# AbrahamSanders/realtime-codec-agent

Hardware: AMD Instinct MI355X
Metric: batch-encode audio-hours/hour (+ xRT and p50 frame-step latency of 1 duplex stream in `duplex`) (higher is better)
Workload: dtype f32; 1 GPU; batch MagiCodec-style encode, 16 kHz stereo, 0.1 s chunks / 2.0 s context, 256 windows per step (BASELINE configs[1]); codebook=131072x16

## Files before the change

realtime_codec_agent_amd/csrc/rca_codec.hip:

```cpp
#include <stdarg.h>

#include <algorithm>
#include <array>
#include <cmath>
#include <map>
#include <type_traits>

#include "rca_common.h"
#include "rca_conv_balance.h"

namespace rca {
thread_local char g_err[512] = {0};
}
using namespace rca;

typedef float f32x16 __attribute__((ext_vector_type(16)));

#define RCA_LAT_MAX_FRAMES 64
#define RCA_LDS_BUDGET (152 * 1024)

typedef float f32x4 __attribute__((ext_vector_type(4)));

struct RowSrc {
    const float* base;
    int C;
    long chan_stride;
    long win_stride;
    int T;
    const long* row_off = nullptr;
    long span = 0;
    __device__ __forceinline__ long off(long b) const {
        return row_off ? row_off[b] : (b % C) * chan_stride + (b / C) * win_stride;
    }
};

__device__ __forceinline__ float lrelu(float v, float slope) { return v >= 0.0f ? v : v * slope; }

template <int KS>
__global__ __launch_bounds__(256) void conv_in_kernel(RowSrc src, const float* __restrict__ w,
// ... 136 lines not shown
        const int d = TR ? -kk : kk - padL;
        return (d >= 0) ? d / S : -((-d + S - 1) / S);
    }
    static constexpr int off(int kp, int half, int U) {
        const int kl = 2 * kp + half, ci = kl / KS, kk = kl % KS;
        const int d = TR ? -kk : kk - padL;
        const int q = q_of(kp, half);
        return (ci * S + (d - q * S)) * U + 1 + q;
    }
    static constexpr int delta(int kp, int U) { return off(kp, 1, U) - off(kp, 0, U); }
    static constexpr int distinct(int k, int KPC, int U) {
        int found[4] = {0, 0, 0, 0};
        int n = 0;
        for (int kp = 0; kp < KPC; ++kp) {
            const int d = delta(kp, U);
            bool seen = false;
            for (int i = 0; i < n; ++i) seen = seen || found[i] == d;
            if (!seen && n < 4) found[n++] = d;
        }
        return found[k < n ? k : n - 1];
    }
    static constexpr int count(int KPC, int U) {
        int found[8] = {0, 0, 0, 0, 0, 0, 0, 0};
        int n = 0;
        for (int kp = 0; kp < KPC; ++kp) {
            const int d = delta(kp, U);
            bool seen = false;
            for (int i = 0; i < n; ++i) seen = seen || found[i] == d;
            if (!seen && n < 8) found[n++] = d;
        }
        return n;
    }
};

#ifndef RCA_CONV_WPB
#define RCA_CONV_WPB 1
#endif
#ifndef RCA_CONV_OCC
#define RCA_CONV_OCC 2
#endif
#ifndef RCA_CONV_PIPE
#define RCA_CONV_PIPE 1
#endif
#ifndef RCA_CONV_PRIO
#define RCA_CONV_PRIO 1
#endif
#ifndef RCA_CONV_ABUF
#define RCA_CONV_ABUF 1
#endif
#ifndef RCA_CONV_EPRIO
#define RCA_CONV_EPRIO 1
#endif
#ifdef RCA_ABL_NOBREAD
#define RCA_ABL_BREAD(x) (slope)
#else
#define RCA_ABL_BREAD(x) (x)
#endif
typedef __bf16 conv_bf16x8 __attribute__((ext_vector_type(8)));
typedef __bf16 conv_bf16x2 __attribute__((ext_vector_type(2)));
__device__ __forceinline__ unsigned conv_pack_bf16x2(float a, float b) {
    const conv_bf16x2 v = {(__bf16)a, (__bf16)b};
    return __builtin_bit_cast(unsigned, v);
}
template <int BF>
__device__ __forceinline__ void conv_split8(const float (&w)[8], uint4& hi, uint4& lo) {
    unsigned ph[4], pl[4];
#pragma unroll
    for (int j = 0; j < 4; ++j) {
        ph[j] = conv_pack_bf16x2(w[2 * j], w[2 * j + 1]);
        pl[j] = BF == 3 ? conv_pack_bf16x2(w[2 * j] - __uint_as_float(ph[j] << 16), w[2 * j + 1] - __uint_as_float(ph[j] & 0xffff0000u)) : 0u;
    }
    hi = make_uint4(ph[0], ph[1], ph[2], ph[3]);
    lo = make_uint4(pl[0], pl[1], pl[2], pl[3]);
}
template <int KS, int S, int CIC, int WM, int WN, int FUSE, int TR, int BF, int FULLC>
__device__ __forceinline__ void conv1d_mfma_body(const float* __restrict__ x, const float* __restrict__ wp,
                                                 const float* __restrict__ bias, float* __restrict__ y,
                                                 int Cin, int Lin, int Cout, int Lout, long Ncols, int nchunks,
                                                 int pre, float slope, FuseIn fin, TrInfo tr, const long wg, const long n_off) {
    constexpr int MT = WM * 32;
    constexpr int NW = WN * 32;
    constexpr int U = ConvLds<S>::stride(NW);
    constexpr int KPC = CIC * KS / 2;
    constexpr int QPC = KPC / 4;
    constexpr int E = (NW + 2) * S;
    constexpr int PW = (S % 2 == 0 && !TR) ? 2 : 1;
    constexpr int RE = (E + 64 * PW - 1) / (64 * PW);
    constexpr int padL = (KS - S + 1) / 2;
    constexpr int BUF = CIC * S * U + 4;
    static_assert((CIC * KS) % 8 == 0, "chunk must hold whole weight quads");

    extern __shared__ __attribute__((aligned(16))) float xs_all[];
#ifdef RCA_CONV_TIMELINE
    long* const tl_buf = rca_prof_buf;
#endif
    RCA_TL_STAMP(tl0);

    const int lane = threadIdx.x & 63;
    const int half = lane >> 5;
    const int wave = __builtin_amdgcn_readfirstlane(threadIdx.x >> 6);
    float* xs = xs_all + wave * 2 * BUF;
    const int n_co_real = (Cout + MT - 1) / MT;
    const int n_co = TR ? n_co_real * tr.s : n_co_real;
    const int xcd = (int)(wg & 7);
    const long seq = wg >> 3;
    const int co_tile_x = __builtin_amdgcn_readfirstlane((int)(seq % n_co));
    const int phase = TR ? co_tile_x / n_co_real : 0;
    const int co_tile = TR ? co_tile_x % n_co_real : co_tile_x;
    const long col_tile = (seq / n_co) * 8 + xcd;
    const long n0 = n_off + (col_tile * RCA_CONV_WPB + wave) * NW;
    const int co0 = co_tile * MT;
    if (n0 >= Ncols) return;
    const long n_base = n0 > 0 ? n0 - 1 : 0;
    const int b_base = __builtin_amdgcn_readfirstlane((int)((unsigned)n_base / (unsigned)Lout));
    const int t_base = (int)(n_base - (long)b_base * Lout);
    const int lead = n0 > 0 ? 0 : 1;
    const long left = Ncols - n_base;
    const int ncol_left = left > NW + 2 ? NW + 2 : (int)left;
    auto rel_bt = [&](int dn, int& bb, int& tt) {
        int dt = dn + t_base;
        bb = 0;
        if (Lout >= NW + 3) {
            if (dt >= Lout) { dt -= Lout; bb = 1; }
        } else {
            bb = dt / Lout;
            dt -= bb * Lout;
        }
        tt = dt;
    };

    constexpr unsigned OOB = 0x80000000u;
    const rca_rsrc_t rs_x = rca_make_rsrc(FUSE ? fin.src.base : x + (long)b_base * Cin * Lin, 0x7FFFFFFF);
// ... 99 lines not shown
    float4 a[WM][QPC];
    if (!FUSE) stage_load(0);
#pragma unroll
    for (int wm = 0; wm < WM; ++wm) {
        const float4* p0 = w_ptr(wm, 0);
#pragma unroll
        for (int q = 0; q < QPC; ++q) a[wm][q] = RCA_CONV_ABUF ? w_load(wm, 0, q) : p0[q * 64];
    }
    __builtin_amdgcn_sched_barrier(0);
    typedef ConvBOff<KS, S, TR> BO;
    static_assert(BO::count(KPC, U) <= 3, "B-operand base registers");
    constexpr int BD0 = BO::distinct(0, KPC, U), BD1 = BO::distinct(1, KPC, U), BD2 = BO::distinct(2, KPC, U);
    const int b_base0 = (lane & 31) + half * BD0, b_base1 = (lane & 31) + half * BD1, b_base2 = (lane & 31) + half * BD2;
    auto b_off = [&](int kp) __attribute__((always_inline)) {
        const int dl = BO::delta(kp, U);
        return (dl == BD0 ? b_base0 : dl == BD1 ? b_base1 : b_base2) + BO::off(kp, 0, U);
    };
    unsigned m_first = 0, m_last = 0;
#pragma unroll
    for (int kp = 0; kp < KPC; ++kp) {
        const int q = half ? BO::q_of(kp, 1) : BO::q_of(kp, 0);
        if (q < 0) m_first |= 1u << kp;
        if (q > 0) m_last |= 1u << kp;
    }
    unsigned zmask[WN];
    unsigned zany = 0;
#pragma unroll
    for (int wn = 0; wn < WN; ++wn) {
        int bz, t;
        rel_bt(1 - lead + wn * 32 + (lane & 31), bz, t);
        zmask[wn] = (t == 0 ? m_first : 0u) | (t == Lout - 1 ? m_last : 0u);
        zany |= zmask[wn];
    }
    const bool edges = __builtin_amdgcn_ballot_w64(zany != 0) != 0;

    f32x16 acc[WM][WN];
#pragma unroll
    for (int wm = 0; wm < WM; ++wm) {
#pragma unroll
        for (int q = 0; q < 4; ++q) {
            const f32x4 bq = *reinterpret_cast<const f32x4*>(bias + co0 + wm * 32 + 8 * q + 4 * half);
#pragma unroll
            for (int j = 0; j < 4; ++j)
#pragma unroll
                for (int wn = 0; wn < WN; ++wn) acc[wm][wn][4 * q + j] = bq[j];
        }
    }

    auto stage_write_t = [&](int buf, auto act_tag) __attribute__((always_inline)) {
        constexpr bool ACT = decltype(act_tag)::value;
#ifdef RCA_ABL_NOWRITE
        return;
#endif
        float* dst = xs + buf * BUF;
#pragma unroll
        for (int cl = 0; cl < CIC; ++cl) {
#pragma unroll
            for (int r = 0; r < RE; ++r) {
                float v[PW];
#pragma unroll
                for (int j = 0; j < PW; ++j) {
                    v[j] = sreg[cl][r][j];
                    if (ACT && !FUSE) v[j] = fmaxf(v[j], v[j] * slope);
                }
                if (U > NW + 2 || 64 * PW * (r + 1) <= E || s_loff[r] >= 0) {
#pragma unroll
                    for (int j = 0; j < PW; ++j) dst[cl * S * U + s_loff[r] + j * U] = v[j];
                }
            }
        }
    };
    auto stage_write = [&](int buf) __attribute__((always_inline)) {
        if (pre & 1) stage_write_t(buf, std::true_type{});
        else stage_write_t(buf, std::false_type{});
    };

    auto compute_t = [&](int buf, int cn, auto edge_tag) __attribute__((always_inline)) {
        constexpr bool EDGE = decltype(edge_tag)::value;
        const float* xb = xs + buf * BUF;
        const float4* pn[WM];
#pragma unroll
        for (int wm = 0; wm < WM; ++wm) pn[wm] = w_ptr(wm, cn);
        constexpr int NB = (KPC * WN > 32) ? ((KPC % 4 == 0) ? 4 : 2) : (KPC * WN == 32 && WN == 4) ? 2 : 1;
        constexpr int PB = KPC / NB;
        static_assert(KPC % NB == 0, "batching");
#pragma unroll
        for (int nb = 0; nb < NB; ++nb) {
            float bv[PB][WN];
#pragma unroll
            for (int i = 0; i < PB; ++i)
#pragma unroll
                for (int wn = 0; wn < WN; ++wn) bv[i][wn] = xb[b_off(nb * PB + i) + wn * 32];
#pragma unroll
            for (int i = 0; i < PB; ++i) {
                const int kp = nb * PB + i;
                float bfr[WN];
#pragma unroll
                for (int wn = 0; wn < WN; ++wn) bfr[wn] = (EDGE && ((zmask[wn] >> kp) & 1u)) ? 0.0f : bv[i][wn];
#pragma unroll
                for (int wm = 0; wm < WM; ++wm) {
                    const float4 q4 = a[wm][kp >> 2];
                    const float av = (kp & 3) == 0 ? q4.x : (kp & 3) == 1 ? q4.y : (kp & 3) == 2 ? q4.z : q4.w;
#pragma unroll
                    for (int wn = 0; wn < WN; ++wn)
                        acc[wm][wn] = __builtin_amdgcn_mfma_f32_32x32x2f32(av, bfr[wn], acc[wm][wn], 0, 0, 0);
                }
                if ((kp & 3) == 3) {
#pragma unroll
                    for (int wm = 0; wm < WM; ++wm) a[wm][kp >> 2] = RCA_CONV_ABUF ? w_load(wm, cn, kp >> 2) : pn[wm][(kp >> 2) * 64];
                }
            }
        }
    };

    constexpr bool PIPE = RCA_CONV_PIPE && !TR && KS == 16 && BF == 0;
    constexpr int RD = KPC >= 8 ? 4 : 2;
    float bhead[RD][WN];
    auto read_head = [&](int buf) __attribute__((always_inline)) {
        const float* xb = xs + buf * BUF;
#pragma unroll
        for (int i = 0; i < RD; ++i)
#pragma unroll
            for (int wn = 0; wn < WN; ++wn) bhead[i][wn] = RCA_ABL_BREAD(xb[b_off(i) + wn * 32]);
    };
    auto compute_p = [&](int buf, int cn, auto edge_tag) __attribute__((always_inline)) {
        constexpr bool EDGE = decltype(edge_tag)::value;
        const float* xb = xs + buf * BUF;
        const float4* pn[WM];
#pragma unroll
        for (int wm = 0; wm < WM; ++wm) pn[wm] = w_ptr(wm, cn);
        float ring[KPC][WN];
#pragma unroll
        for (int i = 0; i < RD; ++i)
#pragma unroll
            for (int wn = 0; wn < WN; ++wn) ring[i][wn] = bhead[i][wn];
#pragma unroll
        for (int kp = 0; kp < KPC; ++kp) {
#if RCA_CONV_PRIO
            if (kp == KPC / 4 && !RCA_CONV_EPRIO) __builtin_amdgcn_s_setprio(1);
            if (kp == KPC / 2) __builtin_amdgcn_s_setprio(2);
            if (kp == 3 * KPC / 4) __builtin_amdgcn_s_setprio(3);
#endif
            if (kp + RD < KPC) {
#pragma unroll
                for (int wn = 0; wn < WN; ++wn) ring[kp + RD][wn] = RCA_ABL_BREAD(xb[b_off(kp + RD) + wn * 32]);
            }
            float bfr[WN];
#pragma unroll
// ... 51 lines not shown
                    const conv_bf16x8 bhv = __builtin_bit_cast(conv_bf16x8, bh[wn]);
                    acc[wm][wn] = __builtin_amdgcn_mfma_f32_32x32x16_bf16(ahv, bhv, acc[wm][wn], 0, 0, 0);
                    if (BF == 3) {
                        acc[wm][wn] = __builtin_amdgcn_mfma_f32_32x32x16_bf16(ahv, __builtin_bit_cast(conv_bf16x8, bl[wn]), acc[wm][wn], 0, 0, 0);
                        acc[wm][wn] = __builtin_amdgcn_mfma_f32_32x32x16_bf16(alv, bhv, acc[wm][wn], 0, 0, 0);
                    }
                }
#pragma unroll
                for (int qq = 0; qq < 2; ++qq) {
                    const int q = 2 * g + qq;
                    if (q < QPC) a[wm][q] = w_load(wm, cn, q);
                }
            }
        }
    };

    if (FUSE) stage_load(0);
    stage_write(0);
    __builtin_amdgcn_wave_barrier();
    if constexpr (PIPE) read_head(0);
    RCA_TL_STAMP(tl1);
#ifdef RCA_CONV_TIMELINE
    long tl_load = 1 << 30, tl_mfma = 0, tl_write = 0;
#endif
    const int lastc = nchunks - 1;
    auto chunk_loop = [&](auto edge_tag, auto act_tag) __attribute__((always_inline)) {
    for (int c = 0; c < nchunks; c += 2) {
        const int c1 = min(c + 1, lastc);
        RCA_TL_STAMP(ta);
        stage_load(c1);
        __builtin_amdgcn_sched_barrier(0);
        RCA_TL_STAMP(tb);
        __builtin_amdgcn_s_setprio(RCA_CONV_EPRIO);
        if constexpr (BF != 0) compute_b(0, c1, edge_tag);
        else if constexpr (PIPE) compute_p(0, c1, edge_tag);
        else compute_t(0, c1, edge_tag);
        __builtin_amdgcn_s_setprio(RCA_CONV_PRIO ? 3 : 2);
        __builtin_amdgcn_sched_barrier(0);
        RCA_TL_STAMP(tc);
        stage_write_t(1, act_tag);
        __builtin_amdgcn_wave_barrier();
        if constexpr (PIPE) {
            read_head(1);
            __builtin_amdgcn_sched_barrier(0);
        }
        RCA_TL_STAMP(td);
        RCA_TL_MIN(tl_load, tb, tc); RCA_TL_ADD(tl_mfma, tb, tc); RCA_TL_ADD(tl_write, tc, td);
        if (c + 1 >= nchunks) break;
        const int c2 = min(c + 2, lastc);
        stage_load(c2);
        __builtin_amdgcn_sched_barrier(0);
        __builtin_amdgcn_s_setprio(RCA_CONV_EPRIO);
        if constexpr (BF != 0) compute_b(1, c2, edge_tag);
        else if constexpr (PIPE) compute_p(1, c2, edge_tag);
        else compute_t(1, c2, edge_tag);
        __builtin_amdgcn_s_setprio(RCA_CONV_PRIO ? 3 : 2);
        __builtin_amdgcn_sched_barrier(0);
        stage_write_t(0, act_tag);
        __builtin_amdgcn_wave_barrier();
        if constexpr (PIPE) {
            read_head(0);
            __builtin_amdgcn_sched_barrier(0);
        }
    }
    };
    if (pre & 1) {
        if (edges) chunk_loop(std::true_type{}, std::true_type{});
        else chunk_loop(std::false_type{}, std::true_type{});
    } else {
        if (edges) chunk_loop(std::true_type{}, std::false_type{});
        else chunk_loop(std::false_type{}, std::false_type{});
    }

    if (RCA_CONV_EPRIO) __builtin_amdgcn_s_setprio(0);
    RCA_TL_STAMP(tl2);
    const long orow = TR ? tr.Lout : Lout;
    const bool full_rows = co0 + MT <= Cout;
    float* const yw = y + ((long)b_base * Cout + co0) * orow;
#pragma unroll
    for (int wn = 0; wn < WN; ++wn) {
        const int dn = 1 - lead + wn * 32 + (lane & 31);
        if (dn >= ncol_left) continue;
        int bb, t;
        rel_bt(dn, bb, t);
        int ocol = t;
        if (TR) {
            ocol = tr.s * t - tr.padL + phase;
            if (ocol < 0 || ocol >= (int)orow) continue;
        }
        const unsigned voff = ((unsigned)bb * (unsigned)(Cout * (int)orow) + (unsigned)ocol + (unsigned)(4 * half) * (unsigned)orow) * 4u;
        if (pre & 2) {
#pragma unroll
            for (int wm = 0; wm < WM; ++wm)
#pragma unroll
                for (int r = 0; r < 16; ++r) acc[wm][wn][r] = fmaxf(acc[wm][wn][r], acc[wm][wn][r] * slope);
        }
        if (full_rows) {
#pragma unroll
            for (int wm = 0; wm < WM; ++wm)
#pragma unroll
                for (int r = 0; r < 16; ++r) {
                    const int cu = wm * 32 + (r & 3) + 8 * (r >> 2);
                    char* const yr = reinterpret_cast<char*>(yw + (long)cu * orow);
                    *reinterpret_cast<float*>(yr + voff) = acc[wm][wn][r];
                }
        } else {
#pragma unroll
            for (int wm = 0; wm < WM; ++wm)
#pragma unroll
                for (int r = 0; r < 16; ++r) {
                    const int cu = wm * 32 + (r & 3) + 8 * (r >> 2);
                    char* const yr = reinterpret_cast<char*>(yw + (long)cu * orow);
                    if (co0 + cu + 4 * half < Cout) *reinterpret_cast<float*>(yr + voff) = acc[wm][wn][r];
                }
        }
    }
#ifdef RCA_CONV_TIMELINE
    if (tl_buf && lane == 0) {
        const long tl3 = (long)wall_clock64();
        const unsigned hw = __builtin_amdgcn_s_getreg((31 << 11) | (0 << 6) | 4);
        const unsigned xcc = __builtin_amdgcn_s_getreg((3 << 11) | (0 << 6) | 20);
        constexpr int region = KS == 4 ? 0 : KS == 8 ? 1 : KS == 10 ? 2 : KS == 16 ? 3 : KS == 3 ? 4 : 5;
        long* o = tl_buf + ((long)region * 65536 + ((blockIdx.x * RCA_CONV_WPB + wave) & 0xFFFF)) * 8;
        o[6] = tl_load | (tl_mfma << 32);
        o[7] = tl_write | ((long)nchunks << 32);
        o[0] = tl0; o[1] = tl1; o[2] = tl2; o[3] = tl3;
        o[4] = (long)hw | ((long)xcc << 32);
        o[5] = (long)KS | ((long)S << 8) | ((long)(WM | (WN << 4)) << 16) | ((long)wave << 24) | ((long)blockIdx.x << 32);
    }
#endif
}

template <int KS, int S, int CIC, int WM, int WN, int FUSE, int TR, int BF = 0, int FULLC = 0>
__global__ __launch_bounds__(64 * RCA_CONV_WPB, (((KS == 8 && CIC == 2) || (KS == 16 && CIC == 1)) && WM * WN < 8) ? 3 : RCA_CONV_OCC) void conv1d_mfma_kernel(const float* __restrict__ x, const float* __restrict__ wp,
                                                          const float* __restrict__ bias, float* __restrict__ y,
                                                          int Cin, int Lin, int Cout, int Lout, long Ncols, int nchunks,
                                                          int pre, float slope, FuseIn fin, TrInfo tr) {
    conv1d_mfma_body<KS, S, CIC, WM, WN, FUSE, TR, BF, FULLC>(x, wp, bias, y, Cin, Lin, Cout, Lout, Ncols, nchunks, pre, slope, fin, tr, blockIdx.x, 0);
}

template <int KS, int S, int CIC, int WM, int WN, int WM2, int WN2, int FULLC>
__global__ __launch_bounds__(64 * RCA_CONV_WPB, (((KS == 8 && CIC == 2) || (KS == 16 && CIC == 1)) && WM * WN < 8) ? 3 : RCA_CONV_OCC) void conv1d_mfma_mixed_kernel(const float* __restrict__ x, const float* __restrict__ wp,
                                                          const float* __restrict__ bias, float* __restrict__ y,
                                                          int Cin, int Lin, int Cout, int Lout, long Ncols, int nchunks,
                                                          int pre, float slope, unsigned n_bulk_wg, long fine_col0) {
    const FuseIn fin{};
    const TrInfo tr{};
    if (blockIdx.x < n_bulk_wg) conv1d_mfma_body<KS, S, CIC, WM, WN, 0, 0, 0, FULLC>(x, wp, bias, y, Cin, Lin, Cout, Lout, Ncols, nchunks, pre, slope, fin, tr, blockIdx.x, 0);
    else conv1d_mfma_body<KS, S, CIC, WM2, WN2, 0, 0, 0, FULLC>(x, wp, bias, y, Cin, Lin, Cout, Lout, Ncols, nchunks, pre, slope, fin, tr, blockIdx.x - n_bulk_wg, fine_col0);
}

template <int NWN, bool PRE>
__global__ __launch_bounds__(64, 2) void conv_first_mfma_kernel(const float* __restrict__ wp, const float* __restrict__ bias,
                                                               float* __restrict__ y, int Cout, int Lout, long Ncols, int post, float slope,
                                                               FuseIn fin) {
    constexpr int NW = NWN * 32;
    constexpr int E = (NW + 2) * 2;
    constexpr int NBLK = 2 * NWN + 1;
    constexpr int RS = 136;
    constexpr int ZERO = 128;
    constexpr int CIN = 32, KQ = CIN / 2;
    extern __shared__ __attribute__((aligned(16))) float ring[];
#ifdef RCA_CONV_TIMELINE
    long* const tl_buf = rca_prof_buf;
#endif
    RCA_TL_STAMP(tl0);
    const int lane = threadIdx.x & 63;
    const int half = lane >> 5, jl = lane & 31;
    const int n_co = Cout / 64;
    const long wg = blockIdx.x;
    const int xcd = (int)(wg & 7);
    const long seq = wg >> 3;
    const int co_tile = __builtin_amdgcn_readfirstlane((int)(seq % n_co));
    const long n0 = ((seq / n_co) * 8 + xcd) * NW;
    const int co0 = co_tile * 64;
    if (n0 >= Ncols) return;
    const long n_base = n0 > 0 ? n0 - 1 : 0;
    const int b_base = __builtin_amdgcn_readfirstlane((int)((unsigned)n_base / (unsigned)Lout));
    const int t_base = (int)(n_base - (long)b_base * Lout);
    const int lead = n0 > 0 ? 0 : 1;
    const long left = Ncols - n_base;
    const int ncol_left = left > NW + 2 ? NW + 2 : (int)left;
// ... 878 lines not shown
        out[d.out_off + i] = v;
    }
}

__global__ __launch_bounds__(256) void transpose_fj_kernel(const float* __restrict__ in, float* __restrict__ out, int B,
                                                           int F, int J) {
    const long idx = (long)blockIdx.x * blockDim.x + threadIdx.x;
    if (idx >= (long)B * J * F) return;
    const int f = (int)(idx % F);
    const long r = idx / F;
    const int j = (int)(r % J);
    const int b = (int)(r / J);
    out[idx] = in[((long)b * F + f) * J + j];
}
__global__ __launch_bounds__(256) void transpose_df_kernel(const float* __restrict__ in, float* __restrict__ out, int B,
                                                           int D, int F) {
    const long idx = (long)blockIdx.x * blockDim.x + threadIdx.x;
    if (idx >= (long)B * D * F) return;
    const int d = (int)(idx % D);
    const long r = idx / D;
    const int f = (int)(r % F);
    const int b = (int)(r / F);
    out[idx] = in[((long)b * D + d) * F + f];
}

struct ConvLayer {
    int cin, cout, k, s, pre, tr;
    float* w = nullptr;
    float* b = nullptr;
    float* bp = nullptr;
    float* wp = nullptr;
    int K = 0, Kpad = 0, cout_pad = 0, nchunks = 0;
    float* wp2 = nullptr;
    int nchunks2 = 0;
    float* wp_tr = nullptr;
    float* w_lat = nullptr;
    int nchunks_tr = 0;
};

#ifdef RCA_CONV_SMALLCHUNK
#define RCA_CIC_K8 2
#define RCA_CIC_K16 1
#else
#define RCA_CIC_K8 4
#define RCA_CIC_K16 2
#endif
#ifndef RCA_CIC_K3
#define RCA_CIC_K3 8
#endif
static int conv_cic(int k, int s) {
    if (k == 4 && s == 2) return 4;
    if (k == 8 && s == 4) return RCA_CIC_K8;
    if (k == 10 && s == 5) return 4;
    if (k == 16 && s == 8) return RCA_CIC_K16;
    if (k == 3 && s == 1) return RCA_CIC_K3;
    return 0;
}
static int conv_cic_ws(int k, int s) {
    if (k == 4 && s == 2) return 16;
    if (k == 8 && s == 4) return 8;
    if (k == 10 && s == 5) return 8;
    if (k == 16 && s == 8) return 4;
    if (k == 3 && s == 1) return 16;
    return 0;
}

#ifndef RCA_BLK_ABL
#define RCA_BLK_ABL 0
#endif
typedef unsigned short conv_bf16raw;
typedef __attribute__((ext_vector_type(4))) unsigned conv_u32x4;
// ... 353 lines not shown

static int upload(const rca_tensor_t* ts, int n, const std::string& name, long numel, float** out) {
    const rca_tensor_t* t = find_tensor(ts, n, name);
    if (!t) return fail(RCA_ERR_MISSING, "tensor '%s' missing", name.c_str());
    if (t->numel != numel) return fail(RCA_ERR_ARG, "tensor '%s': numel %ld, expected %ld", name.c_str(), (long)t->numel, numel);
    if (t->dtype != RCA_F32) return fail(RCA_ERR_ARG, "tensor '%s' must be f32", name.c_str());
    RCA_HIP(hipMalloc((void**)out, (size_t)numel * sizeof(float)));
    RCA_HIP(hipMemcpy(*out, t->data, (size_t)numel * sizeof(float), hipMemcpyHostToDevice));
    return RCA_OK;
}

static int pack_weights_cic(const float* w_host, const ConvLayer& L, int cic, float** out, int* nchunks_out) {
    const int K = L.cin * L.k;
    const int nchunks = (L.cin + cic - 1) / cic;
    const int Kpad = nchunks * cic * L.k;
    const int cout_pad = (L.cout + 127) / 128 * 128;
    const long n = (long)(cout_pad / 32) * (Kpad / 8) * 64 * 4;
    std::vector<float> p((size_t)n, 0.0f);
    for (int cot = 0; cot < cout_pad / 32; ++cot)
        for (int q = 0; q < Kpad / 8; ++q)
            for (int lane = 0; lane < 64; ++lane)
                for (int e = 0; e < 4; ++e) {
                    const int co = cot * 32 + (lane & 31);
                    const int k = 2 * (4 * q + e) + (lane >> 5);
                    float v = 0.0f;
                    if (co < L.cout && k < K) v = w_host[(long)co * K + k];
                    p[(((long)cot * (Kpad / 8) + q) * 64 + lane) * 4 + e] = v;
                }
    RCA_HIP(hipMalloc((void**)out, (size_t)n * sizeof(float)));
    RCA_HIP(hipMemcpy(*out, p.data(), (size_t)n * sizeof(float), hipMemcpyHostToDevice));
    *nchunks_out = nchunks;
    return RCA_OK;
}
static int pack_weights(const float* w_host, ConvLayer& L) {
    L.K = L.cin * L.k;
    L.cout_pad = (L.cout + 127) / 128 * 128;
    int rc = pack_weights_cic(w_host, L, conv_cic(L.k, L.s), &L.wp, &L.nchunks);
    if (rc != RCA_OK) return rc;
    L.Kpad = L.nchunks * conv_cic(L.k, L.s) * L.k;
    return pack_weights_cic(w_host, L, conv_cic_ws(L.k, L.s), &L.wp2, &L.nchunks2);
}

static int pack_weights_tr(const float* w_host, ConvLayer& L) {
    const int cic = 16, K = 2 * L.cin;
    const int nchunks = (L.cin + cic - 1) / cic;
    const int Kpad = nchunks * cic * 2;
    L.cout_pad = (L.cout + 127) / 128 * 128;
    const long per_phase = (long)(L.cout_pad / 32) * (Kpad / 8) * 64 * 4;
    std::vector<float> p((size_t)per_phase * L.s, 0.0f);
    for (int r = 0; r < L.s; ++r)
        for (int cot = 0; cot < L.cout_pad / 32; ++cot)
            for (int q = 0; q < Kpad / 8; ++q)
                for (int lane = 0; lane < 64; ++lane)
                    for (int e = 0; e < 4; ++e) {
                        const int co = cot * 32 + (lane & 31);
                        const int k = 2 * (4 * q + e) + (lane >> 5);
                        float v = 0.0f;
                        if (co < L.cout && k < K) {
                            const int ci = k >> 1, j = k & 1;
                            v = w_host[((long)ci * L.cout + co) * L.k + r + j * L.s];
                        }
                        p[r * per_phase + (((long)cot * (Kpad / 8) + q) * 64 + lane) * 4 + e] = v;
                    }
    RCA_HIP(hipMalloc((void**)&L.wp_tr, p.size() * sizeof(float)));
    RCA_HIP(hipMemcpy(L.wp_tr, p.data(), p.size() * sizeof(float), hipMemcpyHostToDevice));
    {
        std::vector<float> t((size_t)L.cin * L.cout * L.k);
        for (int ci = 0; ci < L.cin; ++ci)
            for (int co = 0; co < L.cout; ++co)
                for (int kk = 0; kk < L.k; ++kk) t[((size_t)co * L.k + kk) * L.cin + ci] = w_host[((size_t)ci * L.cout + co) * L.k + kk];
        RCA_HIP(hipMalloc((void**)&L.w_lat, t.size() * sizeof(float)));
        RCA_HIP(hipMemcpy(L.w_lat, t.data(), t.size() * sizeof(float), hipMemcpyHostToDevice));
// ... 19 lines not shown
    RCA_HIP(hipGetDeviceCount(n));
    return RCA_OK;
}

extern "C" int rca_codec_destroy(rca_codec_t* h) {
#ifdef RCA_CONV_TIMELINE
    if (h && getenv("RCA_CONV_TIMELINE_OUT")) {
        long* b = nullptr;
        unsigned n = 6 << 16;
        (void)hipDeviceSynchronize();
        (void)hipMemcpyFromSymbol(&b, HIP_SYMBOL(rca_prof_buf), 8);
        if (b) {
            std::vector<long> host((size_t)(6 << 16) * 8);
            (void)hipMemcpy(host.data(), b, host.size() * 8, hipMemcpyDeviceToHost);
            if (FILE* f = fopen(getenv("RCA_CONV_TIMELINE_OUT"), "wb")) { fwrite(&n, 4, 1, f); fwrite(host.data(), 8, host.size(), f); fclose(f); }
        }
    }
#endif

    if (!h) return RCA_OK;
    (void)hipSetDevice(h->device);
    for (auto& pk : h->bf16_packs) {
        if (pk.hi) (void)hipFree(pk.hi);
        if (pk.lo) (void)hipFree(pk.lo);
        if (pk.w_in8) (void)hipFree(pk.w_in8);
    }
    for (auto* v : {&h->enc, &h->dec})
        for (auto& L : *v) {
            if (L.w) (void)hipFree(L.w);
            if (L.b) (void)hipFree(L.b);
            if (L.bp) (void)hipFree(L.bp);
            if (L.wp) (void)hipFree(L.wp);
            if (L.wp2) (void)hipFree(L.wp2);
            if (L.wp_tr) (void)hipFree(L.wp_tr);
            if (L.w_lat) (void)hipFree(L.w_lat);
        }
    for (float* p : {h->q_in_w, h->q_in_b, h->cb, h->hc, h->cbp})
        if (p) (void)hipFree(p);
    if (h->err_flag) (void)hipFree(h->err_flag);
    for (auto& kv : h->sgraphs)
        if (kv.second.exec) (void)hipGraphExecDestroy(kv.second.exec);
    if (h->pin) (void)hipHostFree(h->pin);
    for (auto& kv : h->ingest_tabs)
        if (kv.second) (void)hipFree(kv.second);
    h->act[0].release(); h->act[1].release(); h->zbuf.release(); h->keys.release(); h->io_a.release(); h->io_b.release(); h->tail.release();
    for (auto* v : {&h->prof, &h->prof_pool})
        for (auto& p : *v) { (void)hipEventDestroy(p.a); (void)hipEventDestroy(p.b); }
    if (h->xev) (void)hipEventDestroy(h->xev);
    if (h->stream) (void)hipStreamDestroy(h->stream);
    delete h;
    return RCA_OK;
}

static void codec_receptive_field(const rca_codec_config_t& c, int hop, int* enc_left, int* dec_left) {
    const int n = c.n_stages;
    long lo = 0;
    lo = lo - (c.k_latent - 1 + 1) / 2;
    for (int i = n - 1; i >= 0; --i) { const int s = c.strides[i], k = 2 * s; lo = lo * s - (k - s + 1) / 2; }
    lo = lo - (c.k_in - 1 + 1) / 2;
    *enc_left = (int)((-lo + hop - 1) / hop);
    auto ceil_div = [](long a, long b) { return a >= 0 ? (a + b - 1) / b : -((-a) / b); };
    long u = 0;
    u = u - (c.k_in - 1 + 1) / 2;
    for (int i = 0; i < n; ++i) { const int s = c.strides[i], k = 2 * s; u = ceil_div(u + (k - s + 1) / 2 - (k - 1), s); }
    u = u - (c.k_latent - 1 + 1) / 2;
    *dec_left = (int)(-u);
// ... 82 lines not shown
    }
#endif
    codebook_proj_kernel<<<cdiv((long)N * J, 256), 256, 0, h->stream>>>(raw, pw, pb, h->cb, N, R, J);
    codebook_norm_pack_kernel<<<cdiv(N, 256), 256, 0, h->stream>>>(h->cb, h->hc, h->cbp, N, J);
    hipError_t e = hipStreamSynchronize(h->stream);
    free3();
    if (e != hipSuccess) return bail(fail(RCA_ERR_HIP, "codebook init: %s", hipGetErrorString(e)));
    *out = h;
    return RCA_OK;
}

extern "C" int rca_codec_hop(const rca_codec_t* h, int32_t* hop) {
    if (!h || !hop) return fail(RCA_ERR_ARG, "null");
    *hop = h->hop;
    return RCA_OK;
}
extern "C" int rca_codec_num_frames(const rca_codec_t* h, int32_t T, int32_t* F) {
    if (!h || !F || T < 0) return fail(RCA_ERR_ARG, "bad argument");
    *F = (T + h->hop - 1) / h->hop;
    return RCA_OK;
}
extern "C" int rca_codec_set_variant(rca_codec_t* h, int32_t v) {
    if (!h || v < 0 || v > 2) return fail(RCA_ERR_ARG, "variant must be 0, 1 or 2");
    h->variant = v;
    return RCA_OK;
}
extern "C" int rca_codec_sync(rca_codec_t* h) {
    if (!h) return fail(RCA_ERR_ARG, "null");
    RCA_HIP(hipSetDevice(h->device));
    RCA_HIP(hipStreamSynchronize(h->stream));
    return RCA_OK;
}

template <int KS, int S, int CIC, int WM, int WN>
static bool launch_conv_balanced(const ConvLayer& L, const float* wp, int nchunks, const float* x, float* y, int Lin, int Lc, long Ncols,
                                 float slope, hipStream_t st, int act, int lds) {
    constexpr int NT = RCA_CONV_WPB * WN * 32, MT = WM * 32;
    const char* on = getenv("RCA_CONV_BALANCE");
    if (on && on[0] == '0') return false;
    const long total = cdiv(Ncols, NT);
    const int n_co = (int)cdiv(L.cout, MT);
    ConvBalancePlan p;
    if (!conv_balance_parse(getenv("RCA_CONV_BALANCE_PLAN"), total, WM, WN, &p)) {
        static int simds_of[64], occ_of[64];
        int dev = 0;
        if (hipGetDevice(&dev) != hipSuccess || dev < 0 || dev >= 64) return false;
        if (!simds_of[dev]) {
            int cus = 0, blocks = 0;
            if (hipDeviceGetAttribute(&cus, hipDeviceAttributeMultiprocessorCount, dev) != hipSuccess || cus <= 0) return false;
            if (hipOccupancyMaxActiveBlocksPerMultiprocessor(&blocks, conv1d_mfma_kernel<KS, S, CIC, WM, WN, 0, 0, 0, 1>, 64 * RCA_CONV_WPB, lds) != hipSuccess || blocks < 4)
                return false;
            occ_of[dev] = blocks * RCA_CONV_WPB / 4;
            simds_of[dev] = 4 * cus;
        }
        p = conv_balance_plan(total, n_co, simds_of[dev], occ_of[dev], WM, WN);
    }
    if (!p.fine_wn) return false;
    const long fine_col0 = p.bulk_col_tiles * NT;
    const long n_bulk_wg = p.bulk_col_tiles * n_co;
    const long fine_tiles = (cdiv(Ncols - fine_col0, RCA_CONV_WPB * p.fine_wn * 32) + 7) / 8 * 8;
    const long n_wg = n_bulk_wg + fine_tiles * cdiv(L.cout, p.fine_wm * 32);
    if (n_wg >= (1L << 31)) return false;
    const dim3 grid((unsigned)n_wg);
    if (WM * WN == 4 && p.fine_wn == 2)
        conv1d_mfma_mixed_kernel<KS, S, CIC, WM, WN, 1, (WM * WN == 4 ? 2 : 1), 1><<<grid, 64 * RCA_CONV_WPB, lds, st>>>(x, wp, L.bp, y, L.cin, Lin, L.cout, Lc, Ncols, nchunks, act, slope, (unsigned)n_bulk_wg, fine_col0);
    else
        conv1d_mfma_mixed_kernel<KS, S, CIC, WM, WN, 1, 1, 1><<<grid, 64 * RCA_CONV_WPB, lds, st>>>(x, wp, L.bp, y, L.cin, Lin, L.cout, Lc, Ncols, nchunks, act, slope, (unsigned)n_bulk_wg, fine_col0);
    return true;
}

template <int KS, int S, int CIC, int WM, int WN, int FUSE, int TR, int BF = 0>
static void launch_conv_cfg(const ConvLayer& L, const float* wp, int nchunks, const float* x, float* y, int Lin, int Lc, long Ncols,
                            float slope, const FuseIn& fin, const TrInfo& tr, hipStream_t st, int act) {
    constexpr int NT = RCA_CONV_WPB * WN * 32, MT = WM * 32;
    constexpr int lds = RCA_CONV_WPB * 2 * (CIC * S * ConvLds<S>::stride(WN * 32) + 4) * 4;
    static_assert(lds <= 65536, "LDS budget");
    const long col_tiles = (cdiv(Ncols, NT) + 7) / 8 * 8;
    dim3 grid((unsigned)(col_tiles * cdiv(L.cout, MT) * (TR ? tr.s : 1)));
    if constexpr (!FUSE && !TR && BF == 0) {
        if (L.cin % CIC == 0 && nchunks * CIC == L.cin) {
            if constexpr (KS >= 8 && WN == 2 && WM <= 2) {
                if (launch_conv_balanced<KS, S, CIC, WM, WN>(L, wp, nchunks, x, y, Lin, Lc, Ncols, slope, st, act, lds)) return;
            }
            conv1d_mfma_kernel<KS, S, CIC, WM, WN, 0, 0, 0, 1><<<grid, 64 * RCA_CONV_WPB, lds, st>>>(x, wp, L.bp, y, L.cin, Lin, L.cout, Lc, Ncols, nchunks, act, slope, fin, tr);
            return;
        }
    }
    conv1d_mfma_kernel<KS, S, CIC, WM, WN, FUSE, TR, BF><<<grid, 64 * RCA_CONV_WPB, lds, st>>>(x, wp, L.bp, y, L.cin, Lin, L.cout, Lc, Ncols, nchunks, act, slope, fin, tr);
}

template <int KS, int S, int CIC>
static int launch_conv_mfma(const ConvLayer& L, const float* x, float* y, int B, int Lin, int Lout, float slope, hipStream_t st,
                            const FuseIn* fuse = nullptr, int act = -1, int bf = 0) {
    if (act < 0) act = L.pre;
    const long Ncols = (long)B * Lout;
    if (bf) {
        const FuseIn none_b{};
        const TrInfo notr_b{};
        const bool big = (long)cdiv(Ncols, 64) * cdiv(L.cout, 64) >= 2048;
#define RCA_BF_LAUNCH(FU, BFM) do { \
            if (big) launch_conv_cfg<KS, S, CIC, 2, 2, FU, 0, BFM>(L, L.wp, L.nchunks, x, y, Lin, Lout, Ncols, slope, FU ? *fuse : none_b, notr_b, st, act); \
            else launch_conv_cfg<KS, S, CIC, 1, 1, FU, 0, BFM>(L, L.wp, L.nchunks, x, y, Lin, Lout, Ncols, slope, FU ? *fuse : none_b, notr_b, st, act); } while (0)
        if constexpr (KS == 4 || KS == 8 || KS == 16) {
            if (fuse) { if (bf == 3) RCA_BF_LAUNCH(1, 3); else RCA_BF_LAUNCH(1, 1); RCA_LAUNCH_CHECK(); return RCA_OK; }
        }
        if (fuse) return fail(RCA_ERR_ARG, "internal: fused first layer of this shape has no bf16 instantiation");
        if (bf == 3) RCA_BF_LAUNCH(0, 3); else RCA_BF_LAUNCH(0, 1);
#undef RCA_BF_LAUNCH
        RCA_LAUNCH_CHECK();
        return RCA_OK;
    }
    const long waves_big = (long)cdiv(Ncols, 64) * cdiv(L.cout, 64);
#ifdef RCA_CONV_FORCE_MID
// ... 1188 lines not shown
```

Before: 3543 audio-hours/hour.

## Add 16x16x4 f32 MFMA path for strided conv layers with repacked weights

Adds an alternative conv1d MFMA body that uses 16x16x4 f32 instructions instead of 32x32x2, with its own B-operand offset classes, edge masks, accumulator layout, epilogue and a separately packed weight buffer. It is selected by default for the k=10, s=5 layers at WM=WN=2 and can be overridden through an env var. The intent is a better fit between the instruction shape and these layers' LDS operand reuse and edge handling. In exchange it costs extra weight memory, more template instantiations, and possibly different register pressure.

Result: no change. 3545 audio-hours/hour, median of 2 (+0.1%).

```diff
diff --git a/realtime_codec_agent_amd/csrc/rca_codec.hip b/realtime_codec_agent_amd/csrc/rca_codec.hip
--- a/realtime_codec_agent_amd/csrc/rca_codec.hip
+++ b/realtime_codec_agent_amd/csrc/rca_codec.hip
@@ -5,6 +5,7 @@
 #include <cmath>
 #include <map>
 #include <type_traits>
+#include <utility>
 
 #include "rca_common.h"
 #include "rca_conv_balance.h"
@@ -207,6 +208,45 @@
         return n;
     }
 };
+
+template <int KS, int S, int KQC, int U>
+struct ConvBOff16 {
+    typedef ConvBOff<KS, S, 0> BO;
+    static constexpr int MAXC = 5;
+    static constexpr int offk(int k) { return BO::off(k >> 1, k & 1, U); }
+    static constexpr int qk(int k) { return BO::q_of(k >> 1, k & 1); }
+    static constexpr int delta(int kq, int g) { return offk(4 * kq + g) - offk(4 * kq); }
+    static constexpr bool same(int a, int b) { return delta(a, 1) == delta(b, 1) && delta(a, 2) == delta(b, 2) && delta(a, 3) == delta(b, 3); }
+    static constexpr int first(int kq) {
+        for (int i = 0; i < kq; ++i) if (same(i, kq)) return i;
+        return kq;
+    }
+    static constexpr int cls(int kq) {
+        int n = 0;
+        const int f = first(kq);
+        for (int i = 0; i < f; ++i) if (first(i) == i) ++n;
+        return n;
+    }
+    static constexpr int count() {
+        int n = 0;
+        for (int i = 0; i < KQC; ++i) if (first(i) == i) ++n;
+        return n;
+    }
+    static constexpr int rep(int c) {
+        int n = 0, last = 0;
+        for (int i = 0; i < KQC; ++i) if (first(i) == i) { if (n == c) return i; ++n; last = i; }
+        return last;
+    }
+    static constexpr unsigned edge_mask(int g, int sign) {
+        unsigned m = 0;
+        for (int kq = 0; kq < KQC; ++kq) if (sign < 0 ? qk(4 * kq + g) < 0 : qk(4 * kq + g) > 0) m |= 1u << kq;
+        return m;
+    }
+};
+template <class F, int... I>
+__device__ __forceinline__ void conv_static_for_impl(F&& f, std::integer_sequence<int, I...>) { (f(std::integral_constant<int, I>{}), ...); }
+template <int N, class F>
+__device__ __forceinline__ void conv_static_for(F&& f) { conv_static_for_impl(f, std::make_integer_sequence<int, N>{}); }
 
 #ifndef RCA_CONV_WPB
 #define RCA_CONV_WPB 1
@@ -248,7 +288,7 @@
     hi = make_uint4(ph[0], ph[1], ph[2], ph[3]);
     lo = make_uint4(pl[0], pl[1], pl[2], pl[3]);
 }
-template <int KS, int S, int CIC, int WM, int WN, int FUSE, int TR, int BF, int FULLC>
+template <int KS, int S, int CIC, int WM, int WN, int FUSE, int TR, int BF, int FULLC, int SH = 32>
 __device__ __forceinline__ void conv1d_mfma_body(const float* __restrict__ x, const float* __restrict__ wp,
                                                  const float* __restrict__ bias, float* __restrict__ y,
                                                  int Cin, int Lin, int Cout, int Lout, long Ncols, int nchunks,
@@ -264,6 +304,9 @@
     constexpr int padL = (KS - S + 1) / 2;
     constexpr int BUF = CIC * S * U + 4;
     static_assert((CIC * KS) % 8 == 0, "chunk must hold whole weight quads");
+    static_assert(SH == 32 || (SH == 16 && !FUSE && !TR && BF == 0 && FULLC == 1), "the 16x16x4 shape covers the plain f32 path only");
+    constexpr int KQC = KPC / 2;
+    constexpr int WM16 = SH == 16 ? 2 * WM : 1, WN16 = SH == 16 ? 2 * WN : 1;
 
     extern __shared__ __attribute__((aligned(16))) float xs_all[];
 #ifdef RCA_CONV_TIMELINE
@@ -273,6 +316,7 @@
 
     const int lane = threadIdx.x & 63;
     const int half = lane >> 5;
+    const int g16 = lane >> 4;
     const int wave = __builtin_amdgcn_readfirstlane(threadIdx.x >> 6);
     float* xs = xs_all + wave * 2 * BUF;
     const int n_co_real = (Cout + MT - 1) / MT;
@@ -438,11 +482,43 @@
         zmask[wn] = (t == 0 ? m_first : 0u) | (t == Lout - 1 ? m_last : 0u);
         zany |= zmask[wn];
     }
+    typedef ConvBOff16<KS, S, KQC, U> BO16;
+    int b16_base[BO16::MAXC];
+    unsigned zmask16[WN16];
+    if constexpr (SH == 16) {
+        static_assert(BO16::count() <= BO16::MAXC, "B-operand base registers");
+        conv_static_for<BO16::MAXC>([&](auto ic) __attribute__((always_inline)) {
+            constexpr int c = decltype(ic)::value, r = BO16::rep(c);
+            constexpr int d1 = BO16::delta(r, 1), d2 = BO16::delta(r, 2), d3 = BO16::delta(r, 3);
+            b16_base[c] = (lane & 15) + (g16 == 0 ? 0 : g16 == 1 ? d1 : g16 == 2 ? d2 : d3);
+        });
+        constexpr unsigned F0 = BO16::edge_mask(0, -1), F1 = BO16::edge_mask(1, -1), F2 = BO16::edge_mask(2, -1), F3 = BO16::edge_mask(3, -1);
+        constexpr unsigned L0 = BO16::edge_mask(0, 1), L1 = BO16::edge_mask(1, 1), L2 = BO16::edge_mask(2, 1), L3 = BO16::edge_mask(3, 1);
+        const unsigned mf = g16 == 0 ? F0 : g16 == 1 ? F1 : g16 == 2 ? F2 : F3;
+        const unsigned ml = g16 == 0 ? L0 : g16 == 1 ? L1 : g16 == 2 ? L2 : L3;
+        zany = 0;
+#pragma unroll
+        for (int cb = 0; cb < WN16; ++cb) {
+            int bz, t;
+            rel_bt(1 - lead + cb * 16 + (lane & 15), bz, t);
+            zmask16[cb] = (t == 0 ? mf : 0u) | (t == Lout - 1 ? ml : 0u);
+            zany |= zmask16[cb];
+        }
+    }
     const bool edges = __builtin_amdgcn_ballot_w64(zany != 0) != 0;
 
     f32x16 acc[WM][WN];
-#pragma unroll
-    for (int wm = 0; wm < WM; ++wm) {
+    f32x4 acc16[WM16][WN16];
+    if constexpr (SH == 16) {
+#pragma unroll
+        for (int rb = 0; rb < WM16; ++rb) {
+            const f32x4 bq = *reinterpret_cast<const f32x4*>(bias + co0 + rb * 16 + 4 * g16);
+#pragma unroll
+            for (int cb = 0; cb < WN16; ++cb) acc16[rb][cb] = bq;
+        }
+    }
+#pragma unroll
+    for (int wm = 0; wm < (SH == 16 ? 0 : WM); ++wm) {
 #pragma unroll
         for (int q = 0; q < 4; ++q) {
             const f32x4 bq = *reinterpret_cast<const f32x4*>(bias + co0 + wm * 32 + 8 * q + 4 * half);
@@ -487,7 +563,11 @@
         const float4* pn[WM];
 #pragma unroll
         for (int wm = 0; wm < WM; ++wm) pn[wm] = w_ptr(wm, cn);
+#ifdef RCA_ABL_NB2_K10
+        constexpr int NB = (KS == 10 && KPC * WN > 32) ? 2 : (KPC * WN > 32) ? ((KPC % 4 == 0) ? 4 : 2) : (KPC * WN == 32 && WN == 4) ? 2 : 1;
+#else
         constexpr int NB = (KPC * WN > 32) ? ((KPC % 4 == 0) ? 4 : 2) : (KPC * WN == 32 && WN == 4) ? 2 : 1;
+#endif
         constexpr int PB = KPC / NB;
         static_assert(KPC % NB == 0, "batching");
 #pragma unroll
@@ -519,7 +599,43 @@
         }
     };
 
-    constexpr bool PIPE = RCA_CONV_PIPE && !TR && KS == 16 && BF == 0;
+    auto compute_16 = [&](int buf, int cn, auto edge_tag) __attribute__((always_inline)) {
+        constexpr bool EDGE = decltype(edge_tag)::value;
+        const float* xb = xs + buf * BUF;
+        constexpr int NB32 = (KPC * WN > 32) ? ((KPC % 4 == 0) ? 4 : 2) : (KPC * WN == 32 && WN == 4) ? 2 : 1;
+        constexpr int NB = (KQC % NB32 == 0) ? NB32 : (NB32 > 1 && KQC % 2 == 0) ? 2 : 1;
+        constexpr int PQ = KQC / NB;
+        conv_static_for<NB>([&](auto nbc) __attribute__((always_inline)) {
+            constexpr int nb = decltype(nbc)::value;
+            float bv[PQ][WN16];
+            conv_static_for<PQ>([&](auto ic) __attribute__((always_inline)) {
+                constexpr int kq = nb * PQ + decltype(ic)::value;
+                constexpr int o = BO16::offk(4 * kq), c = BO16::cls(kq);
+#pragma unroll
+                for (int cb = 0; cb < WN16; ++cb) bv[decltype(ic)::value][cb] = xb[b16_base[c] + o + cb * 16];
+            });
+            conv_static_for<PQ>([&](auto ic) __attribute__((always_inline)) {
+                constexpr int i = decltype(ic)::value, kq = nb * PQ + i;
+                float bfr[WN16];
+#pragma unroll
+                for (int cb = 0; cb < WN16; ++cb) bfr[cb] = (EDGE && ((zmask16[cb] >> kq) & 1u)) ? 0.0f : bv[i][cb];
+#pragma unroll
+                for (int rb = 0; rb < WM16; ++rb) {
+                    const float4 q4 = a[rb >> 1][kq >> 1];
+                    const float av = (kq & 1) == 0 ? ((rb & 1) == 0 ? q4.x : q4.y) : ((rb & 1) == 0 ? q4.z : q4.w);
+#pragma unroll
+                    for (int cb = 0; cb < WN16; ++cb)
+                        acc16[rb][cb] = __builtin_amdgcn_mfma_f32_16x16x4f32(av, bfr[cb], acc16[rb][cb], 0, 0, 0);
+                }
+                if ((kq & 1) == 1) {
+#pragma unroll
+                    for (int wm = 0; wm < WM; ++wm) a[wm][kq >> 1] = w_load(wm, cn, kq >> 1);
+                }
+            });
+        });
+    };
+
+    constexpr bool PIPE = RCA_CONV_PIPE && !TR && KS == 16 && BF == 0 && SH == 32;
     constexpr int RD = KPC >= 8 ? 4 : 2;
     float bhead[RD][WN];
     auto read_head = [&](int buf) __attribute__((always_inline)) {
@@ -637,7 +753,8 @@
         __builtin_amdgcn_sched_barrier(0);
         RCA_TL_STAMP(tb);
         __builtin_amdgcn_s_setprio(RCA_CONV_EPRIO);
-        if constexpr (BF != 0) compute_b(0, c1, edge_tag);
+        if constexpr (SH == 16) compute_16(0, c1, edge_tag);
+        else if constexpr (BF != 0) compute_b(0, c1, edge_tag);
         else if constexpr (PIPE) compute_p(0, c1, edge_tag);
         else compute_t(0, c1, edge_tag);
         __builtin_amdgcn_s_setprio(RCA_CONV_PRIO ? 3 : 2);
@@ -656,7 +773,8 @@
         stage_load(c2);
         __builtin_amdgcn_sched_barrier(0);
         __builtin_amdgcn_s_setprio(RCA_CONV_EPRIO);
-        if constexpr (BF != 0) compute_b(1, c2, edge_tag);
+        if constexpr (SH == 16) compute_16(1, c2, edge_tag);
+        else if constexpr (BF != 0) compute_b(1, c2, edge_tag);
         else if constexpr (PIPE) compute_p(1, c2, edge_tag);
         else compute_t(1, c2, edge_tag);
         __builtin_amdgcn_s_setprio(RCA_CONV_PRIO ? 3 : 2);
@@ -682,8 +800,43 @@
     const long orow = TR ? tr.Lout : Lout;
     const bool full_rows = co0 + MT <= Cout;
     float* const yw = y + ((long)b_base * Cout + co0) * orow;
-#pragma unroll
-    for (int wn = 0; wn < WN; ++wn) {
+    if constexpr (SH == 16) {
+#pragma unroll
+        for (int cb = 0; cb < WN16; ++cb) {
+            const int dn = 1 - lead + cb * 16 + (lane & 15);
+            if (dn >= ncol_left) continue;
+            int bb, t;
+            rel_bt(dn, bb, t);
+            const unsigned voff = ((unsigned)bb * (unsigned)(Cout * (int)orow) + (unsigned)t + (unsigned)(4 * g16) * (unsigned)orow) * 4u;
+            if (pre & 2) {
+#pragma unroll
+                for (int rb = 0; rb < WM16; ++rb)
+#pragma unroll
+                    for (int r = 0; r < 4; ++r) acc16[rb][cb][r] = fmaxf(acc16[rb][cb][r], acc16[rb][cb][r] * slope);
+            }
+            if (full_rows) {
+#pragma unroll
+                for (int rb = 0; rb < WM16; ++rb)
+#pragma unroll
+                    for (int r = 0; r < 4; ++r) {
+                        const int cu = rb * 16 + r;
+                        char* const yr = reinterpret_cast<char*>(yw + (long)cu * orow);
+                        *reinterpret_cast<float*>(yr + voff) = acc16[rb][cb][r];
+                    }
+            } else {
+#pragma unroll
+                for (int rb = 0; rb < WM16; ++rb)
+#pragma unroll
+                    for (int r = 0; r < 4; ++r) {
+                        const int cu = rb * 16 + r;
+                        char* const yr = reinterpret_cast<char*>(yw + (long)cu * orow);
+                        if (co0 + cu + 4 * g16 < Cout) *reinterpret_cast<float*>(yr + voff) = acc16[rb][cb][r];
+                    }
+            }
+        }
+    }
+#pragma unroll
+    for (int wn = 0; wn < (SH == 16 ? 0 : WN); ++wn) {
         const int dn = 1 - lead + wn * 32 + (lane & 31);
         if (dn >= ncol_left) continue;
         int bb, t;
@@ -736,23 +889,23 @@
 #endif
 }
 
-template <int KS, int S, int CIC, int WM, int WN, int FUSE, int TR, int BF = 0, int FULLC = 0>
+template <int KS, int S, int CIC, int WM, int WN, int FUSE, int TR, int BF = 0, int FULLC = 0, int SH = 32>
 __global__ __launch_bounds__(64 * RCA_CONV_WPB, (((KS == 8 && CIC == 2) || (KS == 16 && CIC == 1)) && WM * WN < 8) ? 3 : RCA_CONV_OCC) void conv1d_mfma_kernel(const float* __restrict__ x, const float* __restrict__ wp,
                                                           const float* __restrict__ bias, float* __restrict__ y,
                                                           int Cin, int Lin, int Cout, int Lout, long Ncols, int nchunks,
                                                           int pre, float slope, FuseIn fin, TrInfo tr) {
-    conv1d_mfma_body<KS, S, CIC, WM, WN, FUSE, TR, BF, FULLC>(x, wp, bias, y, Cin, Lin, Cout, Lout, Ncols, nchunks, pre, slope, fin, tr, blockIdx.x, 0);
-}
-
-template <int KS, int S, int CIC, int WM, int WN, int WM2, int WN2, int FULLC>
+    conv1d_mfma_body<KS, S, CIC, WM, WN, FUSE, TR, BF, FULLC, SH>(x, wp, bias, y, Cin, Lin, Cout, Lout, Ncols, nchunks, pre, slope, fin, tr, blockIdx.x, 0);
+}
+
+template <int KS, int S, int CIC, int WM, int WN, int WM2, int WN2, int FULLC, int SH = 32>
 __global__ __launch_bounds__(64 * RCA_CONV_WPB, (((KS == 8 && CIC == 2) || (KS == 16 && CIC == 1)) && WM * WN < 8) ? 3 : RCA_CONV_OCC) void conv1d_mfma_mixed_kernel(const float* __restrict__ x, const float* __restrict__ wp,
                                                           const float* __restrict__ bias, float* __restrict__ y,
                                                           int Cin, int Lin, int Cout, int Lout, long Ncols, int nchunks,
                                                           int pre, float slope, unsigned n_bulk_wg, long fine_col0) {
     const FuseIn fin{};
     const TrInfo tr{};
-    if (blockIdx.x < n_bulk_wg) conv1d_mfma_body<KS, S, CIC, WM, WN, 0, 0, 0, FULLC>(x, wp, bias, y, Cin, Lin, Cout, Lout, Ncols, nchunks, pre, slope, fin, tr, blockIdx.x, 0);
-    else conv1d_mfma_body<KS, S, CIC, WM2, WN2, 0, 0, 0, FULLC>(x, wp, bias, y, Cin, Lin, Cout, Lout, Ncols, nchunks, pre, slope, fin, tr, blockIdx.x - n_bulk_wg, fine_col0);
+    if (blockIdx.x < n_bulk_wg) conv1d_mfma_body<KS, S, CIC, WM, WN, 0, 0, 0, FULLC, SH>(x, wp, bias, y, Cin, Lin, Cout, Lout, Ncols, nchunks, pre, slope, fin, tr, blockIdx.x, 0);
+    else conv1d_mfma_body<KS, S, CIC, WM2, WN2, 0, 0, 0, FULLC, SH>(x, wp, bias, y, Cin, Lin, Cout, Lout, Ncols, nchunks, pre, slope, fin, tr, blockIdx.x - n_bulk_wg, fine_col0);
 }
 
 template <int NWN, bool PRE>
@@ -1697,11 +1850,19 @@
     float* wp = nullptr;
     int K = 0, Kpad = 0, cout_pad = 0, nchunks = 0;
     float* wp2 = nullptr;
+    float* wp16 = nullptr;
     int nchunks2 = 0;
     float* wp_tr = nullptr;
     float* w_lat = nullptr;
     int nchunks_tr = 0;
 };
+
+static int conv_mfma_shape(const ConvLayer& L, int wm, int wn) {
+    const char* e = getenv("RCA_CONV_MFMA_SHAPE");
+    if (e && e[0] == '1' && e[1] == '6' && !e[2]) return 16;
+    if (e && e[0] == '3' && e[1] == '2' && !e[2]) return 32;
+    return (L.k == 10 && L.s == 5 && wm == 2 && wn == 2) ? 16 : 32;
+}
 
 #ifdef RCA_CONV_SMALLCHUNK
 #define RCA_CIC_K8 2
@@ -2121,12 +2282,37 @@
     *nchunks_out = nchunks;
     return RCA_OK;
 }
+static int pack_weights_sh16(const float* w_host, const ConvLayer& L, int cic, float** out) {
+    const int K = L.cin * L.k;
+    const int nchunks = (L.cin + cic - 1) / cic;
+    const int Kpad = nchunks * cic * L.k;
+    const int cout_pad = (L.cout + 127) / 128 * 128;
+    const long n = (long)(cout_pad / 32) * (Kpad / 8) * 64 * 4;
+    std::vector<float> p((size_t)n, 0.0f);
+    for (int cot = 0; cot < cout_pad / 32; ++cot)
+        for (int q = 0; q < Kpad / 8; ++q)
+            for (int lane = 0; lane < 64; ++lane)
+                for (int e = 0; e < 4; ++e) {
+                    const int co = cot * 32 + (e & 1) * 16 + (lane & 15);
+                    const int k = 8 * q + 4 * (e >> 1) + (lane >> 4);
+                    float v = 0.0f;
+                    if (co < L.cout && k < K) v = w_host[(long)co * K + k];
+                    p[(((long)cot * (Kpad / 8) + q) * 64 + lane) * 4 + e] = v;
+                }
+    RCA_HIP(hipMalloc((void**)out, (size_t)n * sizeof(float)));
+    RCA_HIP(hipMemcpy(*out, p.data(), (size_t)n * sizeof(float), hipMemcpyHostToDevice));
+    return RCA_OK;
+}
 static int pack_weights(const float* w_host, ConvLayer& L) {
     L.K = L.cin * L.k;
     L.cout_pad = (L.cout + 127) / 128 * 128;
     int rc = pack_weights_cic(w_host, L, conv_cic(L.k, L.s), &L.wp, &L.nchunks);
     if (rc != RCA_OK) return rc;
     L.Kpad = L.nchunks * conv_cic(L.k, L.s) * L.k;
+    if (L.k >= 8 && L.s > 1 && L.cin % conv_cic(L.k, L.s) == 0) {
+        rc = pack_weights_sh16(w_host, L, conv_cic(L.k, L.s), &L.wp16);
+        if (rc != RCA_OK) return rc;
+    }
     return pack_weights_cic(w_host, L, conv_cic_ws(L.k, L.s), &L.wp2, &L.nchunks2);
 }
 
@@ -2212,6 +2398,7 @@
             if (L.bp) (void)hipFree(L.bp);
             if (L.wp) (void)hipFree(L.wp);
             if (L.wp2) (void)hipFree(L.wp2);
+            if (L.wp16) (void)hipFree(L.wp16);
             if (L.wp_tr) (void)hipFree(L.wp_tr);
             if (L.w_lat) (void)hipFree(L.w_lat);
         }
@@ -2360,7 +2547,7 @@
     return RCA_OK;
 }
 
-template <int KS, int S, int CIC, int WM, int WN>
+template <int KS, int S, int CIC, int WM, int WN, int SH = 32>
 static bool launch_conv_balanced(const ConvLayer& L, const float* wp, int nchunks, const float* x, float* y, int Lin, int Lc, long Ncols,
                                  float slope, hipStream_t st, int act, int lds) {
     constexpr int NT = RCA_CONV_WPB * WN * 32, MT = WM * 32;
@@ -2376,7 +2563,7 @@
         if (!simds_of[dev]) {
             int cus = 0, blocks = 0;
             if (hipDeviceGetAttribute(&cus, hipDeviceAttributeMultiprocessorCount, dev) != hipSuccess || cus <= 0) return false;
-            if (hipOccupancyMaxActiveBlocksPerMultiprocessor(&blocks, conv1d_mfma_kernel<KS, S, CIC, WM, WN, 0, 0, 0, 1>, 64 * RCA_CONV_WPB, lds) != hipSuccess || blocks < 4)
+            if (hipOccupancyMaxActiveBlocksPerMultiprocessor(&blocks, conv1d_mfma_kernel<KS, S, CIC, WM, WN, 0, 0, 0, 1, SH>, 64 * RCA_CONV_WPB, lds) != hipSuccess || blocks < 4)
                 return false;
             occ_of[dev] = blocks * RCA_CONV_WPB / 4;
             simds_of[dev] = 4 * cus;
@@ -2391,9 +2578,9 @@
     if (n_wg >= (1L << 31)) return false;
     const dim3 grid((unsigned)n_wg);
     if (WM * WN == 4 && p.fine_wn == 2)
-        conv1d_mfma_mixed_kernel<KS, S, CIC, WM, WN, 1, (WM * WN == 4 ? 2 : 1), 1><<<grid, 64 * RCA_CONV_WPB, lds, st>>>(x, wp, L.bp, y, L.cin, Lin, L.cout, Lc, Ncols, nchunks, act, slope, (unsigned)n_bulk_wg, fine_col0);
+        conv1d_mfma_mixed_kernel<KS, S, CIC, WM, WN, 1, (WM * WN == 4 ? 2 : 1), 1, SH><<<grid, 64 * RCA_CONV_WPB, lds, st>>>(x, wp, L.bp, y, L.cin, Lin, L.cout, Lc, Ncols, nchunks, act, slope, (unsigned)n_bulk_wg, fine_col0);
     else
-        conv1d_mfma_mixed_kernel<KS, S, CIC, WM, WN, 1, 1, 1><<<grid, 64 * RCA_CONV_WPB, lds, st>>>(x, wp, L.bp, y, L.cin, Lin, L.cout, Lc, Ncols, nchunks, act, slope, (unsigned)n_bulk_wg, fine_col0);
+        conv1d_mfma_mixed_kernel<KS, S, CIC, WM, WN, 1, 1, 1, SH><<<grid, 64 * RCA_CONV_WPB, lds, st>>>(x, wp, L.bp, y, L.cin, Lin, L.cout, Lc, Ncols, nchunks, act, slope, (unsigned)n_bulk_wg, fine_col0);
     return true;
 }
 
@@ -2407,6 +2594,15 @@
     dim3 grid((unsigned)(col_tiles * cdiv(L.cout, MT) * (TR ? tr.s : 1)));
     if constexpr (!FUSE && !TR && BF == 0) {
         if (L.cin % CIC == 0 && nchunks * CIC == L.cin) {
+            if constexpr (KS >= 8 && WM <= 2 && WN <= 2) {
+                if (wp == L.wp && L.wp16 && conv_mfma_shape(L, WM, WN) == 16) {
+                    if constexpr (WN == 2) {
+                        if (launch_conv_balanced<KS, S, CIC, WM, WN, 16>(L, L.wp16, nchunks, x, y, Lin, Lc, Ncols, slope, st, act, lds)) return;
+                    }
+                    conv1d_mfma_kernel<KS, S, CIC, WM, WN, 0, 0, 0, 1, 16><<<grid, 64 * RCA_CONV_WPB, lds, st>>>(x, L.wp16, L.bp, y, L.cin, Lin, L.cout, Lc, Ncols, nchunks, act, slope, fin, tr);
+                    return;
+                }
+            }
             if constexpr (KS >= 8 && WN == 2 && WM <= 2) {
                 if (launch_conv_balanced<KS, S, CIC, WM, WN>(L, wp, nchunks, x, y, Lin, Lc, Ncols, slope, st, act, lds)) return;
             }
```
